# naver/multi-hmr

Hardware: NVIDIA H100
Metric: images/sec multiHMR_896_L bs=8 (higher is better)
Workload: dtype fp16 tensor-core operands, fp32 accumulate/residual

## Files before the change

### multi-hmr_b200/csrc/common.cuh

```cuda
#pragma once

#include <cuda.h>
#include <cuda_fp16.h>
#include <cuda_runtime.h>
#include <stdint.h>
#include <stdio.h>
#include <string>

#include "../../include/mhmr.h"

namespace mhmr {

__device__ __forceinline__ void griddep_launch_dependents() { asm volatile("griddepcontrol.launch_dependents;" ::: "memory"); }
__device__ __forceinline__ void griddep_wait() { asm volatile("griddepcontrol.wait;" ::: "memory"); }


void set_last_error(const std::string& msg);
const char* get_last_error();

#define MHMR_CUDA_CHECK(expr)                                                          \
  do {                                                                                 \
    cudaError_t _e = (expr);                                                           \
    if (_e != cudaSuccess) {                                                           \
      ::mhmr::set_last_error(std::string(#expr) + " failed: " + cudaGetErrorString(_e) + \
                             " at " + __FILE__ + ":" + std::to_string(__LINE__));      \
      return MHMR_ERR_CUDA;                                                    \
    }                                                                                  \
  } while (0)

#define MHMR_REQUIRE(cond, msg)                                                        \
  do {                                                                                 \
    if (!(cond)) {                                                                     \
      ::mhmr::set_last_error(std::string("requirement failed: ") + #cond + " — " + msg); \
      return MHMR_ERR_ARG;                                                     \
    }                                                                                  \
  } while (0)

#define TRY(...)                    \
  do {                              \
    int rc_ = (__VA_ARGS__);        \
    if (rc_ != MHMR_OK) return rc_; \
  } while (0)

int make_tmap_2d(CUtensorMap* out, const void* gptr, CUtensorMapDataType dtype, int elem_bytes,
                 uint64_t rows, uint64_t cols, uint64_t pitch_bytes, uint32_t box_rows,
                 uint32_t box_cols, bool swizzle128);
int make_tmap_3d(CUtensorMap* out, const void* gptr, CUtensorMapDataType dtype, int elem_bytes,
                 uint64_t depth, uint64_t rows, uint64_t cols, uint64_t depth_pitch_bytes, uint64_t pitch_bytes,
                 uint32_t box_rows, uint32_t box_cols, bool swizzle128);

int device_sm_count();
struct PerDeviceOnce {
  bool done[64] = {};
  bool first();
};
bool pdl_enabled();

#ifdef __CUDACC__
__device__ __forceinline__ uint32_t smem_u32(const void* p) {
  return static_cast<uint32_t>(__cvta_generic_to_shared(p));
}
__device__ __forceinline__ uint32_t lane_id() { return threadIdx.x & 31u; }
__device__ __forceinline__ bool elect_one_sync() {
  uint32_t pred = 0;
  asm volatile(
      "{\n\t.reg .b32 rx;\n\t.reg .pred px;\n\t"
      "elect.sync rx|px, %1;\n\t"
      "selp.u32 %0, 1, 0, px;\n\t}"
      : "=r"(pred)
      : "r"(0xffffffffu));
  return pred != 0;
}

__device__ __forceinline__ void mbar_init(uint64_t* bar, uint32_t count) {
  asm volatile("mbarrier.init.shared::cta.b64 [%0], %1;" ::"r"(smem_u32(bar)), "r"(count));
}
__device__ __forceinline__ void fence_barrier_init() {
  asm volatile("fence.mbarrier_init.release.cluster;" ::: "memory");
}
__device__ __forceinline__ void fence_proxy_async_smem() {
  asm volatile("fence.proxy.async.shared::cta;" ::: "memory");
}
__device__ __forceinline__ void mbar_arrive_expect_tx(uint64_t* bar, uint32_t bytes) {
  asm volatile("mbarrier.arrive.expect_tx.shared::cta.b64 _, [%0], %1;" ::"r"(smem_u32(bar)),
               "r"(bytes)
               : "memory");
}
__device__ __forceinline__ void mbar_arrive(uint64_t* bar) {
  asm volatile("mbarrier.arrive.shared::cta.b64 _, [%0];" ::"r"(smem_u32(bar)) : "memory");
}
__device__ __forceinline__ bool mbar_try_wait(uint64_t* bar, uint32_t parity) {
  uint32_t ok;
  asm volatile(
      "{\n\t.reg .pred p;\n\t"
      "mbarrier.try_wait.parity.shared::cta.b64 p, [%1], %2;\n\t"
      "selp.u32 %0, 1, 0, p;\n\t}"
      : "=r"(ok)
      : "r"(smem_u32(bar)), "r"(parity)
      : "memory");
  return ok != 0;
}
#ifndef MHMR_SPIN_LIMIT
#define MHMR_SPIN_LIMIT (1u << 28)
#endif
__device__ __forceinline__ void mbar_wait(uint64_t* bar, uint32_t parity) {
  uint32_t spins = 0;
  while (!mbar_try_wait(bar, parity)) {
    if (++spins > MHMR_SPIN_LIMIT) __trap();
  }
}

__device__ __forceinline__ void tma_prefetch_desc(const CUtensorMap* tmap) {
  asm volatile("prefetch.tensormap [%0];" ::"l"(reinterpret_cast<uint64_t>(tmap)) : "memory");
}
__device__ __forceinline__ void tma_load_2d(void* smem_dst, const CUtensorMap* tmap, uint64_t* bar,
                                            int32_t c_inner, int32_t c_outer) {
  asm volatile(
      "cp.async.bulk.tensor.2d.shared::cluster.global.mbarrier::complete_tx::bytes"
      " [%0], [%1, {%3, %4}], [%2];"
      :
      : "r"(smem_u32(smem_dst)), "l"(reinterpret_cast<uint64_t>(tmap)), "r"(smem_u32(bar)),
        "r"(c_inner), "r"(c_outer)
      : "memory");
}
__device__ __forceinline__ void tma_load_2d_hint(void* smem_dst, const CUtensorMap* tmap,
                                                 uint64_t* bar, int32_t c_inner, int32_t c_outer,
                                                 uint64_t cache_hint) {
  asm volatile(
      "cp.async.bulk.tensor.2d.shared::cluster.global.mbarrier::complete_tx::bytes.L2::cache_hint"
      " [%0], [%1, {%3, %4}], [%2], %5;"
      :
      : "r"(smem_u32(smem_dst)), "l"(reinterpret_cast<uint64_t>(tmap)), "r"(smem_u32(bar)),
        "r"(c_inner), "r"(c_outer), "l"(cache_hint)
      : "memory");
}
__device__ __forceinline__ void tma_load_3d_hint(void* smem_dst, const CUtensorMap* tmap, uint64_t* bar,
                                                 int32_t c_inner, int32_t c_row, int32_t c_depth,
                                                 uint64_t cache_hint) {
  asm volatile(
      "cp.async.bulk.tensor.3d.shared::cluster.global.mbarrier::complete_tx::bytes.L2::cache_hint"
      " [%0], [%1, {%3, %4, %5}], [%2], %6;"
      :
      : "r"(smem_u32(smem_dst)), "l"(reinterpret_cast<uint64_t>(tmap)), "r"(smem_u32(bar)),
        "r"(c_inner), "r"(c_row), "r"(c_depth), "l"(cache_hint)
      : "memory");
}
__device__ __forceinline__ void tma_store_2d(const CUtensorMap* tmap, const void* smem_src,
                                             int32_t c_inner, int32_t c_outer) {
  asm volatile("cp.async.bulk.tensor.2d.global.shared::cta.bulk_group [%0, {%2, %3}], [%1];"
               :
               : "l"(reinterpret_cast<uint64_t>(tmap)), "r"(smem_u32(smem_src)), "r"(c_inner),
                 "r"(c_outer)
               : "memory");
}
__device__ __forceinline__ void tma_store_commit() {
  asm volatile("cp.async.bulk.commit_group;" ::: "memory");
}
template <int N>
__device__ __forceinline__ void tma_store_wait_read() {
  asm volatile("cp.async.bulk.wait_group.read %0;" ::"n"(N) : "memory");
}
template <int N>
__device__ __forceinline__ void tma_store_wait() {
  asm volatile("cp.async.bulk.wait_group %0;" ::"n"(N) : "memory");
}
constexpr uint64_t kCacheEvictFirst = 0x12F0000000000000ull;
constexpr uint64_t kCacheEvictLast = 0x14F0000000000000ull;
constexpr uint64_t kCacheEvictNormal = 0x1000000000000000ull;

__device__ __forceinline__ uint32_t cluster_ctarank() {
  uint32_t r;
  asm volatile("mov.u32 %0, %%cluster_ctarank;" : "=r"(r));
  return r;
}
__device__ __forceinline__ void cluster_sync_all() {
  asm volatile("barrier.cluster.arrive.release.aligned;" ::: "memory");
  asm volatile("barrier.cluster.wait.acquire.aligned;" ::: "memory");
}
__device__ __forceinline__ void mbar_arrive_remote(uint64_t* bar, uint32_t cta) {
  uint32_t remote;
  asm volatile("mapa.shared::cluster.u32 %0, %1, %2;" : "=r"(remote) : "r"(smem_u32(bar)), "r"(cta));
  asm volatile("mbarrier.arrive.shared::cluster.b64 _, [%0];" ::"r"(remote) : "memory");
}
__device__ __forceinline__ void tma_load_2d_multicast(void* smem_dst, const CUtensorMap* tmap, uint64_t* bar,
                                                      int32_t c_inner, int32_t c_outer, uint16_t cta_mask) {
  asm volatile(
      "cp.async.bulk.tensor.2d.shared::cluster.global.mbarrier::complete_tx::bytes.multicast::cluster"
      " [%0], [%1, {%3, %4}], [%2], %5;"
      :
      : "r"(smem_u32(smem_dst)), "l"(reinterpret_cast<uint64_t>(tmap)), "r"(smem_u32(bar)),
        "r"(c_inner), "r"(c_outer), "h"(cta_mask)
      : "memory");
}

__device__ __forceinline__ uint64_t make_sw128_desc(uint32_t smem_addr, uint32_t lbo_bytes,
                                                    uint32_t sbo_bytes) {
  uint64_t d = 0;
  d |= static_cast<uint64_t>((smem_addr & 0x3FFFFu) >> 4);
  d |= static_cast<uint64_t>((lbo_bytes >> 4) & 0x3FFFu) << 16;
  d |= static_cast<uint64_t>((sbo_bytes >> 4) & 0x3FFFu) << 32;
  d |= 1ull << 62;
  return d;
}
__device__ __forceinline__ void wgmma_fence() { asm volatile("wgmma.fence.sync.aligned;" ::: "memory"); }
__device__ __forceinline__ void wgmma_commit() { asm volatile("wgmma.commit_group.sync.aligned;" ::: "memory"); }
template <int N>
__device__ __forceinline__ void wgmma_wait() {
  asm volatile("wgmma.wait_group.sync.aligned %0;" ::"n"(N) : "memory");
}
__device__ __forceinline__ void named_bar_sync(uint32_t id, uint32_t count) {
  asm volatile("bar.sync %0, %1;" ::"r"(id), "r"(count) : "memory");
}
__device__ __forceinline__ void named_bar_arrive(uint32_t id, uint32_t count) {
  asm volatile("bar.arrive %0, %1;" ::"r"(id), "r"(count) : "memory");
}
template <int R>
__device__ __forceinline__ void wgmma_fence_regs(float (&d)[R]) {
#pragma unroll
  for (int i = 0; i < R; ++i) asm volatile("" : "+f"(d[i])::"memory");
}

#define MHMR_WG_D8(o) "+f"(d[o + 0]), "+f"(d[o + 1]), "+f"(d[o + 2]), "+f"(d[o + 3]), \
                      "+f"(d[o + 4]), "+f"(d[o + 5]), "+f"(d[o + 6]), "+f"(d[o + 7])
__device__ __forceinline__ void wgmma_m64n64_ss(float (&d)[32], uint64_t da, uint64_t db, uint32_t acc) {
  asm volatile(
      "{\n\t.reg .pred p;\n\tsetp.ne.b32 p, %34, 0;\n\t"
      "wgmma.mma_async.sync.aligned.m64n64k16.f32.f16.f16 "
      "{%0, %1, %2, %3, %4, %5, %6, %7, %8, %9, %10, %11, %12, %13, %14, %15, "
      "%16, %17, %18, %19, %20, %21, %22, %23, %24, %25, %26, %27, %28, %29, %30, %31}, "
      "%32, %33, p, 1, 1, 0, 0;\n\t}"
      : MHMR_WG_D8(0), MHMR_WG_D8(8), MHMR_WG_D8(16), MHMR_WG_D8(24)
      : "l"(da), "l"(db), "r"(acc));
}
__device__ __forceinline__ void wgmma_m64n32_ss(float (&d)[16], uint64_t da, uint64_t db, uint32_t acc) {
  asm volatile(
      "{\n\t.reg .pred p;\n\tsetp.ne.b32 p, %18, 0;\n\t"
      "wgmma.mma_async.sync.aligned.m64n32k16.f32.f16.f16 "
      "{%0, %1, %2, %3, %4, %5, %6, %7, %8, %9, %10, %11, %12, %13, %14, %15}, "
      "%16, %17, p, 1, 1, 0, 0;\n\t}"
      : MHMR_WG_D8(0), MHMR_WG_D8(8)
      : "l"(da), "l"(db), "r"(acc));
}
__device__ __forceinline__ void wgmma_m64n128_ss(float (&d)[64], uint64_t da, uint64_t db, uint32_t acc) {
  asm volatile(
      "{\n\t.reg .pred p;\n\tsetp.ne.b32 p, %66, 0;\n\t"
      "wgmma.mma_async.sync.aligned.m64n128k16.f32.f16.f16 "
      "{%0, %1, %2, %3, %4, %5, %6, %7, %8, %9, %10, %11, %12, %13, %14, %15, "
      "%16, %17, %18, %19, %20, %21, %22, %23, %24, %25, %26, %27, %28, %29, %30, %31, "
      "%32, %33, %34, %35, %36, %37, %38, %39, %40, %41, %42, %43, %44, %45, %46, %47, "
      "%48, %49, %50, %51, %52, %53, %54, %55, %56, %57, %58, %59, %60, %61, %62, %63}, "
      "%64, %65, p, 1, 1, 0, 0;\n\t}"
      : MHMR_WG_D8(0), MHMR_WG_D8(8), MHMR_WG_D8(16), MHMR_WG_D8(24), MHMR_WG_D8(32), MHMR_WG_D8(40),
        MHMR_WG_D8(48), MHMR_WG_D8(56)
      : "l"(da), "l"(db), "r"(acc));
}
__device__ __forceinline__ void wgmma_m64n64_rs_bt(float (&d)[32], const uint32_t (&a)[4], uint64_t db) {
  asm volatile(
      "{\n\t.reg .pred p;\n\tsetp.ne.b32 p, 1, 0;\n\t"
      "wgmma.mma_async.sync.aligned.m64n64k16.f32.f16.f16 "
      "{%0, %1, %2, %3, %4, %5, %6, %7, %8, %9, %10, %11, %12, %13, %14, %15, "
      "%16, %17, %18, %19, %20, %21, %22, %23, %24, %25, %26, %27, %28, %29, %30, %31}, "
      "{%32, %33, %34, %35}, %36, p, 1, 1, 1;\n\t}"
      : MHMR_WG_D8(0), MHMR_WG_D8(8), MHMR_WG_D8(16), MHMR_WG_D8(24)
      : "r"(a[0]), "r"(a[1]), "r"(a[2]), "r"(a[3]), "l"(db));
}
#undef MHMR_WG_D8

__device__ __forceinline__ float2 fma2(float2 a, float2 b, float2 c) {
  return make_float2(fmaf(a.x, b.x, c.x), fmaf(a.y, b.y, c.y));
}
__device__ __forceinline__ float2 mul2(float2 a, float2 b) { return make_float2(__fmul_rn(a.x, b.x), __fmul_rn(a.y, b.y)); }
__device__ __forceinline__ float2 add2(float2 a, float2 b) { return make_float2(__fadd_rn(a.x, b.x), __fadd_rn(a.y, b.y)); }

__device__ __forceinline__ float gelu_erf(float x) {
  return 0.5f * x * (1.0f + erff(x * 0.70710678118654752440f));
}

__device__ __forceinline__ float gelu_erf_fast(float x) {
  const float z = fabsf(x) * 0.70710678118654752440f;
  float t;
  asm("rcp.approx.ftz.f32 %0, %1;" : "=f"(t) : "f"(fmaf(0.3275911f, z, 1.0f)));
  float e;
  asm("ex2.approx.ftz.f32 %0, %1;" : "=f"(e) : "f"(-(z * z) * 1.4426950408889634f));
  float p = fmaf(1.061405429f, t, -1.453152027f);
  p = fmaf(p, t, 1.421413741f);
  p = fmaf(p, t, -0.284496736f);
  p = fmaf(p, t, 0.254829592f);
  const float erf_abs = fmaf(-p * t, e, 1.0f);
  return 0.5f * x * (1.0f + copysignf(erf_abs, x));
}

__device__ __forceinline__ float2 gelu_erf_fast2(float2 x) {
  const float2 ax = make_float2(fabsf(x.x), fabsf(x.y));
  const float2 z = mul2(ax, make_float2(0.70710678118654752440f, 0.70710678118654752440f));
  const float2 d = fma2(z, make_float2(0.3275911f, 0.3275911f), make_float2(1.0f, 1.0f));
  float2 t, e;
  asm("rcp.approx.ftz.f32 %0, %1;" : "=f"(t.x) : "f"(d.x));
  asm("rcp.approx.ftz.f32 %0, %1;" : "=f"(t.y) : "f"(d.y));
  const float2 a = mul2(mul2(z, z), make_float2(-1.4426950408889634f, -1.4426950408889634f));
  asm("ex2.approx.ftz.f32 %0, %1;" : "=f"(e.x) : "f"(a.x));
  asm("ex2.approx.ftz.f32 %0, %1;" : "=f"(e.y) : "f"(a.y));
  float2 p = fma2(make_float2(1.061405429f, 1.061405429f), t, make_float2(-1.453152027f, -1.453152027f));
  p = fma2(p, t, make_float2(1.421413741f, 1.421413741f));
  p = fma2(p, t, make_float2(-0.284496736f, -0.284496736f));
  p = fma2(p, t, make_float2(0.254829592f, 0.254829592f));
  const float2 pte = mul2(mul2(p, t), e);
  const float2 erf_abs = fma2(pte, make_float2(-1.0f, -1.0f), make_float2(1.0f, 1.0f));
  const float2 s = make_float2(copysignf(erf_abs.x, x.x), copysignf(erf_abs.y, x.y));
  const float2 hx = mul2(x, make_float2(0.5f, 0.5f));
  return fma2(hx, s, hx);
}

__device__ __forceinline__ float warp_sum(float v) {
#pragma unroll
  for (int o = 16; o > 0; o >>= 1) v += __shfl_xor_sync(0xffffffffu, v, o);
  return v;
}
__device__ __forceinline__ float warp_max(float v) {
#pragma unroll
  for (int o = 16; o > 0; o >>= 1) v = fmaxf(v, __shfl_xor_sync(0xffffffffu, v, o));
  return v;
}
#endif

}
```

### multi-hmr_b200/csrc/gemm_epilogue.cuh

```cuda
#pragma once
#include "gemm_tc.cuh"

namespace mhmr {

constexpr int kScratchStride = 36;
constexpr int kScratchBytes = 32 * kScratchStride * 4;


struct EpiRowState {
  float sum[4], sq[4];
  float rstd;
};

template <int EPI>
constexpr bool epi_is_ln_consumer() { return EPI == EPI_LN_BIAS_F16 || EPI == EPI_LN_GELU_F16; }

struct EpiStatsPrefetch {
  float4 v[4];
};
constexpr int kMaxStatSlots = 8;

template <int EPI>
__device__ __forceinline__ void epilogue_load_row_stats(EpiStatsPrefetch& pf, const GemmEpi& ep, int M, int m_base,
                                                        int lane) {
  if constexpr (epi_is_ln_consumer<EPI>()) {
    const int m = m_base + lane;
    const float4* p = reinterpret_cast<const float4*>(ep.stats + static_cast<int64_t>(m) * ep.stat_slots);
    const int n4 = (m < M) ? (ep.stat_slots >> 1) : 0;
#pragma unroll
    for (int i = 0; i < 4; ++i) pf.v[i] = (i < n4) ? __ldcg(p + i) : make_float4(0.f, 0.f, 0.f, 0.f);
  }
}

template <int EPI>
__device__ __forceinline__ void epilogue_tile_begin(EpiRowState& st, const EpiStatsPrefetch& pf, const GemmEpi& ep,
                                                    int K) {
  if constexpr (EPI == EPI_LS_RESID_SPLIT) {
#pragma unroll
    for (int k = 0; k < 4; ++k) st.sum[k] = st.sq[k] = 0.f;
  }
  if constexpr (epi_is_ln_consumer<EPI>()) {
    const float s = (pf.v[0].x + pf.v[0].z) + (pf.v[1].x + pf.v[1].z) + (pf.v[2].x + pf.v[2].z) + (pf.v[3].x + pf.v[3].z);
    const float q = (pf.v[0].y + pf.v[0].w) + (pf.v[1].y + pf.v[1].w) + (pf.v[2].y + pf.v[2].w) + (pf.v[3].y + pf.v[3].w);
    const float inv = 1.0f / static_cast<float>(K);
    const float mean = s * inv;
    const float var = fmaxf(q * inv - mean * mean, 0.f);
    st.rstd = rsqrtf(var + ep.ln_eps);
  }
}

template <int EPI>
__device__ __forceinline__ void epilogue_tile_end(EpiRowState& st, const GemmEpi& ep, int M, int m_base, int slot,
                                                  int lane) {
  if constexpr (EPI == EPI_LS_RESID_SPLIT) {
    const int cg = lane & 3, rs = lane >> 2;
    const bool h2 = cg & 2, h1 = cg & 1;
#pragma unroll
    for (int i = 0; i < 2; ++i) {
      const float ss = h2 ? st.sum[i] : st.sum[i + 2], ks = h2 ? st.sum[i + 2] : st.sum[i];
      const float sq = h2 ? st.sq[i] : st.sq[i + 2], kq = h2 ? st.sq[i + 2] : st.sq[i];
      st.sum[i] = ks + __shfl_xor_sync(0xffffffffu, ss, 2);
      st.sq[i] = kq + __shfl_xor_sync(0xffffffffu, sq, 2);
    }
    {
      const float ss = h1 ? st.sum[0] : st.sum[1], ks = h1 ? st.sum[1] : st.sum[0];
      const float sq = h1 ? st.sq[0] : st.sq[1], kq = h1 ? st.sq[1] : st.sq[0];
      st.sum[0] = ks + __shfl_xor_sync(0xffffffffu, ss, 1);
      st.sq[0] = kq + __shfl_xor_sync(0xffffffffu, sq, 1);
    }
    const int m = m_base + cg * 8 + rs;
    if (m < M) ep.stats[static_cast<int64_t>(m) * ep.stat_slots + slot] = make_float2(st.sum[0], st.sq[0]);
  }
}

__device__ __forceinline__ void unpack_half8(const uint4& u, float (&f)[8]) {
  const __half2* h = reinterpret_cast<const __half2*>(&u);
#pragma unroll
  for (int i = 0; i < 4; ++i) {
    const float2 t = __half22float2(h[i]);
    f[2 * i] = t.x;
    f[2 * i + 1] = t.y;
  }
}

template <int EPI>
__device__ __forceinline__ void epilogue_chunk(const float* scratch, const GemmEpi& ep, int M, int N, int m_base,
                                               int n0, int lane, EpiRowState& st) {
  constexpr bool kLn = epi_is_ln_consumer<EPI>();
  constexpr bool kRowAdd16 = (EPI == EPI_ROWADD_F16);
  constexpr bool kF16 = (EPI == EPI_BIAS_F16 || EPI == EPI_BIAS_GELU_F16 || EPI == EPI_BIAS_RELU_F16 || kLn || kRowAdd16);
  constexpr bool kResid = (EPI == EPI_LS_RESID_F32);
  if constexpr (EPI == EPI_LS_RESID_SPLIT) {
    const int cg = lane & 3, rs = lane >> 2;
    const int n = n0 + cg * 8;
    float bb[8], gg[8];
    *reinterpret_cast<float4*>(bb) = __ldg(reinterpret_cast<const float4*>(ep.bias + n));
    *reinterpret_cast<float4*>(bb + 4) = __ldg(reinterpret_cast<const float4*>(ep.bias + n + 4));
    *reinterpret_cast<float4*>(gg) = __ldg(reinterpret_cast<const float4*>(ep.gamma + n));
    *reinterpret_cast<float4*>(gg + 4) = __ldg(reinterpret_cast<const float4*>(ep.gamma + n + 4));
    uint4 hi[4], lo[4];
#pragma unroll
    for (int k = 0; k < 4; ++k) {
      const int m = m_base + k * 8 + rs;
      const int64_t off = static_cast<int64_t>(m) * ep.ldx16 + n;
      hi[k] = lo[k] = make_uint4(0u, 0u, 0u, 0u);
      if (m < M) {
        hi[k] = *reinterpret_cast<const uint4*>(ep.x16 + off);
        lo[k] = *reinterpret_cast<const uint4*>(ep.xlo + off);
      }
    }
#pragma unroll
    for (int k = 0; k < 4; ++k) {
      const int rl = k * 8 + rs;
      float v[8], xh[8], xl[8], a[8];
      *reinterpret_cast<float4*>(v) = *reinterpret_cast<const float4*>(scratch + rl * kScratchStride + cg * 8);
      *reinterpret_cast<float4*>(v + 4) = *reinterpret_cast<const float4*>(scratch + rl * kScratchStride + cg * 8 + 4);
      unpack_half8(hi[k], xh);
      unpack_half8(lo[k], xl);
      float s = 0.f, q = 0.f;
      uint32_t ph[4], pl[4];
#pragma unroll
      for (int i = 0; i < 8; ++i) {
        a[i] = fmaf(gg[i], v[i] + bb[i], xh[i] + xl[i]);
        s += a[i];
        q = fmaf(a[i], a[i], q);
      }
#pragma unroll
      for (int i = 0; i < 4; ++i) {
        const __half2 h = __floats2half2_rn(a[2 * i], a[2 * i + 1]);
        const float2 hf = __half22float2(h);
        const __half2 l = __floats2half2_rn(a[2 * i] - hf.x, a[2 * i + 1] - hf.y);
        ph[i] = *reinterpret_cast<const uint32_t*>(&h);
        pl[i] = *reinterpret_cast<const uint32_t*>(&l);
      }
      st.sum[k] += s;
      st.sq[k] += q;
      if (m_base + rl < M) {
        const int64_t off = static_cast<int64_t>(m_base + rl) * ep.ldx16 + n;
        *reinterpret_cast<uint4*>(ep.x16 + off) = make_uint4(ph[0], ph[1], ph[2], ph[3]);
        *reinterpret_cast<uint4*>(ep.xlo + off) = make_uint4(pl[0], pl[1], pl[2], pl[3]);
      }
    }
  } else if constexpr (kF16) {
    const int cg = lane & 3, rs = lane >> 2;
    const int n = n0 + cg * 8;
    float4 b0 = make_float4(0.f, 0.f, 0.f, 0.f), b1 = b0;
    if constexpr (!kRowAdd16) {
      b0 = __ldg(reinterpret_cast<const float4*>(ep.bias + n));
      b1 = __ldg(reinterpret_cast<const float4*>(ep.bias + n + 4));
    }
#pragma unroll
    for (int k = 0; k < 4; ++k) {
      const int rl = k * 8 + rs;
      const int m = m_base + rl;
      if constexpr (kRowAdd16) {
        if (m < M) {
          const float* ra = ep.rowadd + static_cast<int64_t>(m % ep.rows_in) * N + n;
          b0 = __ldg(reinterpret_cast<const float4*>(ra));
          b1 = __ldg(reinterpret_cast<const float4*>(ra + 4));
        }
      }
      const float4 v0 = *reinterpret_cast<const float4*>(scratch + rl * kScratchStride + cg * 8);
      const float4 v1 = *reinterpret_cast<const float4*>(scratch + rl * kScratchStride + cg * 8 + 4);
      float2 y[4];
      if constexpr (kLn) {
        const float rstd = __shfl_sync(0xffffffffu, st.rstd, rl);
        const float2 r2 = make_float2(rstd, rstd);
        y[0] = fma2(make_float2(v0.x, v0.y), r2, make_float2(b0.x, b0.y));
        y[1] = fma2(make_float2(v0.z, v0.w), r2, make_float2(b0.z, b0.w));
        y[2] = fma2(make_float2(v1.x, v1.y), r2, make_float2(b1.x, b1.y));
        y[3] = fma2(make_float2(v1.z, v1.w), r2, make_float2(b1.z, b1.w));
      } else {
        y[0] = add2(make_float2(v0.x, v0.y), make_float2(b0.x, b0.y));
        y[1] = add2(make_float2(v0.z, v0.w), make_float2(b0.z, b0.w));
        y[2] = add2(make_float2(v1.x, v1.y), make_float2(b1.x, b1.y));
        y[3] = add2(make_float2(v1.z, v1.w), make_float2(b1.z, b1.w));
      }
#pragma unroll
      for (int i = 0; i < 4; ++i) {
        if constexpr (EPI == EPI_BIAS_GELU_F16 || EPI == EPI_LN_GELU_F16) y[i] = gelu_erf_fast2(y[i]);
        if constexpr (EPI == EPI_BIAS_RELU_F16) y[i] = make_float2(fmaxf(y[i].x, 0.0f), fmaxf(y[i].y, 0.0f));
      }
      const float x[8] = {y[0].x, y[0].y, y[1].x, y[1].y, y[2].x, y[2].y, y[3].x, y[3].y};
      const __half2 h0 = __floats2half2_rn(x[0], x[1]), h1 = __floats2half2_rn(x[2], x[3]);
      const __half2 h2 = __floats2half2_rn(x[4], x[5]), h3 = __floats2half2_rn(x[6], x[7]);
      uint4 pk;
      pk.x = *reinterpret_cast<const uint32_t*>(&h0);
      pk.y = *reinterpret_cast<const uint32_t*>(&h1);
      pk.z = *reinterpret_cast<const uint32_t*>(&h2);
      pk.w = *reinterpret_cast<const uint32_t*>(&h3);
      if (m < M)
        *reinterpret_cast<uint4*>(reinterpret_cast<__half*>(ep.out) + static_cast<int64_t>(m) * ep.ldo + n) = pk;
    }
  } else {
    const int cg = lane & 7, rs = lane >> 3;
    const int n = n0 + cg * 4;
    float4 b = make_float4(0.f, 0.f, 0.f, 0.f), g = make_float4(1.f, 1.f, 1.f, 1.f);
    if constexpr (kResid) {
      b = __ldg(reinterpret_cast<const float4*>(ep.bias + n));
      g = __ldg(reinterpret_cast<const float4*>(ep.gamma + n));
    } else if constexpr (EPI == EPI_BIAS_F32) {
      if (ep.bias != nullptr) b = __ldg(reinterpret_cast<const float4*>(ep.bias + n));
    }
    float* outp[8];
    float4 xres[8];
#pragma unroll
    for (int k = 0; k < 8; ++k) {
      const int m = m_base + k * 4 + rs;
      int64_t orow = m;
      if constexpr (EPI == EPI_ROWADD_F32) {
        const int grp = m / ep.rows_in, rin = m - grp * ep.rows_in;
        orow = static_cast<int64_t>(grp) * ep.rows_out + ep.row_off + rin;
        xres[k] = (m < M) ? __ldg(reinterpret_cast<const float4*>(ep.rowadd + static_cast<int64_t>(rin) * N + n))
                          : make_float4(0.f, 0.f, 0.f, 0.f);
      }
      outp[k] = reinterpret_cast<float*>(ep.out) + orow * ep.ldo + n;
      if constexpr (kResid)
        xres[k] = (m < M) ? *reinterpret_cast<const float4*>(outp[k]) : make_float4(0.f, 0.f, 0.f, 0.f);
    }
#pragma unroll
    for (int k = 0; k < 8; ++k) {
      const int rl = k * 4 + rs;
      const float4 v = *reinterpret_cast<const float4*>(scratch + rl * kScratchStride + cg * 4);
      float4 a;
      if constexpr (kResid) {
        a.x = xres[k].x + g.x * (v.x + b.x);
        a.y = xres[k].y + g.y * (v.y + b.y);
        a.z = xres[k].z + g.z * (v.z + b.z);
        a.w = xres[k].w + g.w * (v.w + b.w);
      } else if constexpr (EPI == EPI_ROWADD_F32) {
        a.x = v.x + xres[k].x; a.y = v.y + xres[k].y; a.z = v.z + xres[k].z; a.w = v.w + xres[k].w;
      } else {
        a.x = v.x + b.x; a.y = v.y + b.y; a.z = v.z + b.z; a.w = v.w + b.w;
      }
      if (m_base + rl < M) *reinterpret_cast<float4*>(outp[k]) = a;
    }
  }
  __syncwarp();
}

}
```

### multi-hmr_b200/csrc/gemm_tc.cu

```cuda
#include "gemm_tc.cuh"
#include "gemm_epilogue.cuh"

namespace mhmr {

namespace {

constexpr int BM = 128;
constexpr int BK = 64;
constexpr int kConsumers = 2;
constexpr int kThreads = 128 * (1 + kConsumers);
constexpr int kEpiWarps = 4 * kConsumers;
constexpr int kRegsProducer = 40, kRegsConsumer = 232;

template <int BN>
struct GemmCfg {
  static constexpr int kStages = (BN == 256) ? 3 : 5;
  static constexpr int kABytes = BM * BK * 2;
  static constexpr int kBBytes = BN * BK * 2;
  static constexpr int kStageBytes = kABytes + kBBytes;
  static constexpr int kBarBytes = 256;
  static constexpr int kSmemBytes =
      kStages * kStageBytes + kEpiWarps * kScratchBytes + kBarBytes + 1024;
  static constexpr int kAcc = BN / 4;
};

template <int NACC>
__device__ __forceinline__ void wgmma_ss(float (&d)[NACC], uint64_t da, uint64_t db, uint32_t acc) {
  if constexpr (NACC == 64) wgmma_m64n128_ss(d, da, db, acc);
  else wgmma_m64n64_ss(d, da, db, acc);
}

template <int BN, int CL, int EPI>
__global__ void __launch_bounds__(kThreads, 1)
gemm_tc_kernel(const __grid_constant__ CUtensorMap tmA, const __grid_constant__ CUtensorMap tmB,
               int M, int N, int K, GemmEpi ep) {
  using Cfg = GemmCfg<BN>;
  constexpr int kStages = Cfg::kStages;
  constexpr int kAcc = Cfg::kAcc;

  extern __shared__ uint8_t smem_raw[];
  uint8_t* smem = smem_raw + ((1024u - (smem_u32(smem_raw) & 1023u)) & 1023u);
  float* scratch_base = reinterpret_cast<float*>(smem + kStages * Cfg::kStageBytes);
  uint64_t* bars = reinterpret_cast<uint64_t*>(smem + kStages * Cfg::kStageBytes + kEpiWarps * kScratchBytes);
  uint64_t* full_bar = bars;
  uint64_t* empty_bar = bars + kStages;

  const int warp = threadIdx.x >> 5;
  const int lane = threadIdx.x & 31;
  const int wg = threadIdx.x >> 7;
  const uint32_t rank = (CL > 1) ? cluster_ctarank() : 0u;

  const int num_m = (M + BM * CL - 1) / (BM * CL);
  const int num_n = (N + BN - 1) / BN;
  const int num_tiles = num_m * num_n;
  const int num_kb = (K + BK - 1) / BK;
  const int first_tile = blockIdx.x / CL, tile_stride = gridDim.x / CL;

  griddep_launch_dependents();
  if (threadIdx.x == 0) {
    tma_prefetch_desc(&tmA);
    tma_prefetch_desc(&tmB);
    for (int s = 0; s < kStages; ++s) {
      mbar_init(&full_bar[s], 1);
      mbar_init(&empty_bar[s], kConsumers * CL);
    }
    fence_barrier_init();
  }
  if constexpr (CL > 1) cluster_sync_all();
  else __syncthreads();
  griddep_wait();

  if (wg == 0) {
    asm volatile("setmaxnreg.dec.sync.aligned.u32 %0;" ::"n"(kRegsProducer));
    if (warp == 0) {
      uint32_t stage = 0, phase = 0;
      for (int tile = first_tile; tile < num_tiles; tile += tile_stride) {
        const int m_blk = tile / num_n, n_blk = tile % num_n;
        const int row0 = m_blk * BM * CL + static_cast<int>(rank) * BM;
        for (int kb = 0; kb < num_kb; ++kb) {
          mbar_wait(&empty_bar[stage], phase ^ 1u);
          uint8_t* sa = smem + stage * Cfg::kStageBytes;
          uint8_t* sb = sa + Cfg::kABytes;
          if (elect_one_sync()) {
            mbar_arrive_expect_tx(&full_bar[stage], Cfg::kStageBytes);
            tma_load_2d(sa, &tmA, &full_bar[stage], kb * BK, row0);
            if constexpr (CL > 1) {
              constexpr int kHalf = BN / CL;
              tma_load_2d_multicast(sb + rank * (kHalf * BK * 2), &tmB, &full_bar[stage], kb * BK,
                                    n_blk * BN + static_cast<int>(rank) * kHalf, static_cast<uint16_t>((1u << CL) - 1u));
            } else {
              tma_load_2d(sb, &tmB, &full_bar[stage], kb * BK, n_blk * BN);
            }
          }
          __syncwarp();
          if (++stage == kStages) { stage = 0; phase ^= 1u; }
        }
      }
    }
  } else {
    asm volatile("setmaxnreg.inc.sync.aligned.u32 %0;" ::"n"(kRegsConsumer));
    const int cw = wg - 1;
    const int w = warp & 3;
    const bool release_lane = (threadIdx.x & 127) == 0;
    float* scratch = scratch_base + (warp - 4) * (kScratchBytes / 4);
    auto release = [&](uint32_t s) {
      if (release_lane) {
        mbar_arrive(&empty_bar[s]);
        if constexpr (CL > 1) {
#pragma unroll
          for (int c = 0; c < CL; ++c)
            if (c != static_cast<int>(rank)) mbar_arrive_remote(&empty_bar[s], static_cast<uint32_t>(c));
        }
      }
    };
    uint32_t stage = 0, phase = 0;
    EpiStatsPrefetch pf;
    auto tile_m_base = [&](int tile) { return (tile / num_n) * BM * CL + static_cast<int>(rank) * BM + 32 * w; };
    if (first_tile < num_tiles) epilogue_load_row_stats<EPI>(pf, ep, M, tile_m_base(first_tile), lane);
    for (int tile = first_tile; tile < num_tiles; tile += tile_stride) {
      const int n_blk = tile % num_n;
      const int m_base = tile_m_base(tile);
      EpiRowState rowst;
      epilogue_tile_begin<EPI>(rowst, pf, ep, K);
      if (tile + tile_stride < num_tiles)
        epilogue_load_row_stats<EPI>(pf, ep, M, tile_m_base(tile + tile_stride), lane);

      float acc[2][kAcc];
      uint32_t prev_stage = 0;
      for (int kb = 0; kb < num_kb; ++kb) {
        mbar_wait(&full_bar[stage], phase);
        const uint32_t sa = smem_u32(smem + stage * Cfg::kStageBytes);
        const uint32_t sb = sa + Cfg::kABytes + cw * (BN / 2) * (BK * 2);
        const uint64_t a_desc0 = make_sw128_desc(sa, 16, 2048);
        const uint64_t a_desc1 = make_sw128_desc(sa + 1024, 16, 2048);
        const uint64_t b_desc = make_sw128_desc(sb, 16, 1024);
        wgmma_fence();
#pragma unroll
        for (int k = 0; k < BK / 16; ++k) {
          const uint32_t accumulate = (kb > 0 || k > 0) ? 1u : 0u;
          wgmma_ss<kAcc>(acc[0], a_desc0 + 2u * k, b_desc + 2u * k, accumulate);
          wgmma_ss<kAcc>(acc[1], a_desc1 + 2u * k, b_desc + 2u * k, accumulate);
        }
        wgmma_commit();
        wgmma_wait<1>();
        if (kb > 0) release(prev_stage);
        prev_stage = stage;
        if (++stage == kStages) { stage = 0; phase ^= 1u; }
      }
      wgmma_wait<0>();
      wgmma_fence_regs(acc[0]);
      wgmma_fence_regs(acc[1]);
      release(prev_stage);

#pragma unroll
      for (int c = 0; c < BN / 64; ++c) {
#pragma unroll
        for (int h = 0; h < 2; ++h)
#pragma unroll
          for (int g = 0; g < 4; ++g)
#pragma unroll
            for (int rr = 0; rr < 2; ++rr) {
              const int i = 4 * (4 * c + g) + 2 * rr;
              const int r = (lane >> 2) + 8 * h + 16 * rr;
              *reinterpret_cast<float2*>(scratch + r * kScratchStride + g * 8 + 2 * (lane & 3)) =
                  make_float2(acc[h][i], acc[h][i + 1]);
            }
        __syncwarp();
        const int n0 = n_blk * BN + cw * (BN / 2) + c * 32;
        if (n0 < N) epilogue_chunk<EPI>(scratch, ep, M, N, m_base, n0, lane, rowst);
        __syncwarp();
      }
      epilogue_tile_end<EPI>(rowst, ep, M, m_base, n_blk * kConsumers + cw, lane);
    }
  }
  if constexpr (CL > 1) cluster_sync_all();
}

template <int BN, int CL, int EPI>
int launch_one(const GemmPlan* p, cudaStream_t stream) {
  using Cfg = GemmCfg<BN>;
  auto kern = gemm_tc_kernel<BN, CL, EPI>;
  static PerDeviceOnce once;
  if (once.first()) {
    MHMR_CUDA_CHECK(cudaFuncSetAttribute(kern, cudaFuncAttributeMaxDynamicSharedMemorySize,
                                         Cfg::kSmemBytes));
  }
  cudaLaunchConfig_t cfg{};
  cfg.gridDim = dim3(p->grid);
  cfg.blockDim = dim3(kThreads);
  cfg.dynamicSmemBytes = Cfg::kSmemBytes;
  cfg.stream = stream;
  cudaLaunchAttribute attr[2];
  int n = 0;
  if (CL > 1) {
    attr[n].id = cudaLaunchAttributeClusterDimension;
    attr[n].val.clusterDim.x = CL;
    attr[n].val.clusterDim.y = 1;
    attr[n].val.clusterDim.z = 1;
    ++n;
  }
  if (pdl_enabled()) {
    attr[n].id = cudaLaunchAttributeProgrammaticStreamSerialization;
    attr[n].val.programmaticStreamSerializationAllowed = 1;
    ++n;
  }
  cfg.attrs = attr;
  cfg.numAttrs = n;
  MHMR_CUDA_CHECK(cudaLaunchKernelEx(&cfg, kern, p->tmA, p->tmB, p->M, p->N, p->K, p->ep));
  return MHMR_OK;
}

template <int BN, int CL>
int launch_bn(const GemmPlan* p, cudaStream_t stream) {
  switch (p->epi) {
    case EPI_BIAS_F16: return launch_one<BN, CL, EPI_BIAS_F16>(p, stream);
    case EPI_BIAS_GELU_F16: return launch_one<BN, CL, EPI_BIAS_GELU_F16>(p, stream);
    case EPI_BIAS_RELU_F16: return launch_one<BN, CL, EPI_BIAS_RELU_F16>(p, stream);
    case EPI_LS_RESID_F32: return launch_one<BN, CL, EPI_LS_RESID_F32>(p, stream);
    case EPI_ROWADD_F32: return launch_one<BN, CL, EPI_ROWADD_F32>(p, stream);
    case EPI_BIAS_F32: return launch_one<BN, CL, EPI_BIAS_F32>(p, stream);
    case EPI_LS_RESID_SPLIT: return launch_one<BN, CL, EPI_LS_RESID_SPLIT>(p, stream);
    case EPI_LN_BIAS_F16: return launch_one<BN, CL, EPI_LN_BIAS_F16>(p, stream);
    case EPI_LN_GELU_F16: return launch_one<BN, CL, EPI_LN_GELU_F16>(p, stream);
    case EPI_ROWADD_F16: return launch_one<BN, CL, EPI_ROWADD_F16>(p, stream);
    default: break;
  }
  set_last_error("gemm: unknown epilogue kind");
  return MHMR_ERR_ARG;
}

}

int gemm_plan_init(GemmPlan* plan, const __half* A, int64_t lda, const __half* W, int64_t ldw, int M,
                   int N, int K, int epi_kind, const GemmEpi& ep, int bn) {
  MHMR_REQUIRE(M > 0 && N > 0 && K > 0, "gemm: empty problem");
  MHMR_REQUIRE(N % 32 == 0, "gemm: N must be a multiple of 32");
  MHMR_REQUIRE(lda % 8 == 0 && ldw % 8 == 0, "gemm: row pitches must be multiples of 8 fp16 (16 B, TMA)");
  MHMR_REQUIRE((reinterpret_cast<uintptr_t>(A) & 15) == 0 && (reinterpret_cast<uintptr_t>(W) & 15) == 0,
               "gemm: operands must be 16-byte aligned");
  MHMR_REQUIRE(bn == 128 || bn == 256 || bn == 512, "gemm: block_n must be 128, 256 or 512 (CTA pair)");
  MHMR_REQUIRE(epi_kind >= 0 && epi_kind < EPI_NUM_KINDS, "gemm: bad epilogue kind");
  if (epi_kind != EPI_LS_RESID_SPLIT)
    MHMR_REQUIRE(ep.out != nullptr && ep.ldo % 8 == 0, "gemm: output missing or pitch not multiple of 8");
  if (epi_kind != EPI_BIAS_F32 && epi_kind != EPI_ROWADD_F32 && epi_kind != EPI_ROWADD_F16)
    MHMR_REQUIRE(ep.bias != nullptr, "gemm: bias required for this epilogue");
  if (epi_kind == EPI_LS_RESID_F32 || epi_kind == EPI_LS_RESID_SPLIT)
    MHMR_REQUIRE(ep.gamma != nullptr, "gemm: gamma required");
  if (epi_kind == EPI_LS_RESID_SPLIT)
    MHMR_REQUIRE(ep.x16 != nullptr && ep.xlo != nullptr && ep.ldx16 % 8 == 0 && ep.stats != nullptr &&
                     ep.stat_slots == gemm_stat_slots(N, bn) && N % (bn == 128 ? 128 : 256) == 0,
                 "gemm: split-stream epilogue needs both planes, stats, whole column tiles and matching slot count");
  if (epi_kind == EPI_LN_BIAS_F16 || epi_kind == EPI_LN_GELU_F16)
    MHMR_REQUIRE(ep.stats != nullptr && ep.stat_slots > 0 && ep.stat_slots % 2 == 0 && ep.stat_slots <= 8,
                 "gemm: folded-LN consumer needs row statistics (even slot count, at most 8)");
  if (epi_kind == EPI_ROWADD_F32 || epi_kind == EPI_ROWADD_F16)
    MHMR_REQUIRE(ep.rowadd != nullptr && ep.rows_in > 0, "gemm: rowadd/rows_in required");
  plan->M = M; plan->N = N; plan->K = K; plan->bn = bn; plan->epi = epi_kind; plan->ep = ep;
  int rc = make_tmap_2d(&plan->tmA, A, CU_TENSOR_MAP_DATA_TYPE_FLOAT16, 2, M, K, lda * 2, BM, BK, true);
  if (rc != MHMR_OK) return rc;
  rc = make_tmap_2d(&plan->tmB, W, CU_TENSOR_MAP_DATA_TYPE_FLOAT16, 2, N, K, ldw * 2, bn == 512 ? 128 : bn, BK,
                    true);
  if (rc != MHMR_OK) return rc;
  plan->grid = gemm_plan_grid(plan, M);
  return MHMR_OK;
}

int gemm_plan_grid(const GemmPlan* plan, int M) {
  const int sms = device_sm_count();
  if (plan->bn == 512) {
    const int tiles = ((M + 255) / 256) * ((plan->N + 255) / 256);
    const int pairs = sms / 2;
    return 2 * (tiles < pairs ? tiles : pairs);
  }
  const int tiles = ((M + BM - 1) / BM) * ((plan->N + plan->bn - 1) / plan->bn);
  return tiles < sms ? tiles : sms;
}

int gemm_stat_slots(int N, int bn) {
  const int tile_n = (bn == 128) ? 128 : 256;
  return ((N + tile_n - 1) / tile_n) * kConsumers;
}

int gemm_plan_run(const GemmPlan* plan, cudaStream_t stream) {
  if (plan->bn == 512) return launch_bn<256, 2>(plan, stream);
  return plan->bn == 256 ? launch_bn<256, 1>(plan, stream) : launch_bn<128, 1>(plan, stream);
}

int gemm_plan_run_rows(const GemmPlan* plan, int M, cudaStream_t stream) {
  MHMR_REQUIRE(M > 0 && M <= plan->M, "gemm: a plan runs at most the rows it was built for");
  GemmPlan p = *plan;
  p.M = M;
  p.grid = gemm_plan_grid(&p, M);
  return gemm_plan_run(&p, stream);
}

}
```

Baseline: 80.19.

## Split GEMM tile across consumers by rows with one wide wgmma per consumer

Each consumer warpgroup now owns 64 rows across the full BN width and issues a single m64nBNk16 wgmma per k-step, instead of splitting columns and issuing two m64n(BN/2) wgmmas over 128 rows. The epilogue is reworked for 16-row warp slices, and the per-row LayerNorm statistic slots are remapped to two per tile. The intent is fewer, wider wgmma instructions that reuse the A fragment better and lower issue overhead. In exchange the B tile is read by both consumers, and the epilogue and stats bookkeeping change, which risks register pressure and correctness in the split-stat path.

After: 81.11, median of 6. +1.1%, better.

```diff
diff --git a/multi-hmr_b200/csrc/common.cuh b/multi-hmr_b200/csrc/common.cuh
--- a/multi-hmr_b200/csrc/common.cuh
+++ b/multi-hmr_b200/csrc/common.cuh
@@ -252,6 +252,24 @@
       "%64, %65, p, 1, 1, 0, 0;\n\t}"
       : MHMR_WG_D8(0), MHMR_WG_D8(8), MHMR_WG_D8(16), MHMR_WG_D8(24), MHMR_WG_D8(32), MHMR_WG_D8(40),
         MHMR_WG_D8(48), MHMR_WG_D8(56)
+      : "l"(da), "l"(db), "r"(acc));
+}
+__device__ __forceinline__ void wgmma_m64n256_ss(float (&d)[128], uint64_t da, uint64_t db, uint32_t acc) {
+  asm volatile(
+      "{\n\t.reg .pred p;\n\tsetp.ne.b32 p, %130, 0;\n\t"
+      "wgmma.mma_async.sync.aligned.m64n256k16.f32.f16.f16 "
+      "{%0, %1, %2, %3, %4, %5, %6, %7, %8, %9, %10, %11, %12, %13, %14, %15, "
+      "%16, %17, %18, %19, %20, %21, %22, %23, %24, %25, %26, %27, %28, %29, %30, %31, "
+      "%32, %33, %34, %35, %36, %37, %38, %39, %40, %41, %42, %43, %44, %45, %46, %47, "
+      "%48, %49, %50, %51, %52, %53, %54, %55, %56, %57, %58, %59, %60, %61, %62, %63, "
+      "%64, %65, %66, %67, %68, %69, %70, %71, %72, %73, %74, %75, %76, %77, %78, %79, "
+      "%80, %81, %82, %83, %84, %85, %86, %87, %88, %89, %90, %91, %92, %93, %94, %95, "
+      "%96, %97, %98, %99, %100, %101, %102, %103, %104, %105, %106, %107, %108, %109, %110, %111, "
+      "%112, %113, %114, %115, %116, %117, %118, %119, %120, %121, %122, %123, %124, %125, %126, %127}, "
+      "%128, %129, p, 1, 1, 0, 0;\n\t}"
+      : MHMR_WG_D8(0), MHMR_WG_D8(8), MHMR_WG_D8(16), MHMR_WG_D8(24), MHMR_WG_D8(32), MHMR_WG_D8(40),
+        MHMR_WG_D8(48), MHMR_WG_D8(56), MHMR_WG_D8(64), MHMR_WG_D8(72), MHMR_WG_D8(80), MHMR_WG_D8(88),
+        MHMR_WG_D8(96), MHMR_WG_D8(104), MHMR_WG_D8(112), MHMR_WG_D8(120)
       : "l"(da), "l"(db), "r"(acc));
 }
 __device__ __forceinline__ void wgmma_m64n64_rs_bt(float (&d)[32], const uint32_t (&a)[4], uint64_t db) {
diff --git a/multi-hmr_b200/csrc/gemm_epilogue.cuh b/multi-hmr_b200/csrc/gemm_epilogue.cuh
--- a/multi-hmr_b200/csrc/gemm_epilogue.cuh
+++ b/multi-hmr_b200/csrc/gemm_epilogue.cuh
@@ -3,8 +3,9 @@
 
 namespace mhmr {
 
+constexpr int kEpiRows = 16;
 constexpr int kScratchStride = 36;
-constexpr int kScratchBytes = 32 * kScratchStride * 4;
+constexpr int kScratchBytes = kEpiRows * kScratchStride * 4;
 
 
 struct EpiRowState {
@@ -24,7 +25,7 @@
 __device__ __forceinline__ void epilogue_load_row_stats(EpiStatsPrefetch& pf, const GemmEpi& ep, int M, int m_base,
                                                         int lane) {
   if constexpr (epi_is_ln_consumer<EPI>()) {
-    const int m = m_base + lane;
+    const int m = m_base + (lane & (kEpiRows - 1));
     const float4* p = reinterpret_cast<const float4*>(ep.stats + static_cast<int64_t>(m) * ep.stat_slots);
     const int n4 = (m < M) ? (ep.stat_slots >> 1) : 0;
 #pragma unroll
@@ -50,7 +51,7 @@
 }
 
 template <int EPI>
-__device__ __forceinline__ void epilogue_tile_end(EpiRowState& st, const GemmEpi& ep, int M, int m_base, int slot,
+__device__ __forceinline__ void epilogue_tile_end(EpiRowState& st, const GemmEpi& ep, int M, int m_base, int slot0,
                                                   int lane) {
   if constexpr (EPI == EPI_LS_RESID_SPLIT) {
     const int cg = lane & 3, rs = lane >> 2;
@@ -68,8 +69,8 @@
       st.sum[0] = ks + __shfl_xor_sync(0xffffffffu, ss, 1);
       st.sq[0] = kq + __shfl_xor_sync(0xffffffffu, sq, 1);
     }
-    const int m = m_base + cg * 8 + rs;
-    if (m < M) ep.stats[static_cast<int64_t>(m) * ep.stat_slots + slot] = make_float2(st.sum[0], st.sq[0]);
+    const int m = m_base + (cg & 1) * 8 + rs;
+    if (m < M) ep.stats[static_cast<int64_t>(m) * ep.stat_slots + slot0 + (cg >> 1)] = make_float2(st.sum[0], st.sq[0]);
   }
 }
 
@@ -85,7 +86,7 @@
 
 template <int EPI>
 __device__ __forceinline__ void epilogue_chunk(const float* scratch, const GemmEpi& ep, int M, int N, int m_base,
-                                               int n0, int lane, EpiRowState& st) {
+                                               int n0, int half, int lane, EpiRowState& st) {
   constexpr bool kLn = epi_is_ln_consumer<EPI>();
   constexpr bool kRowAdd16 = (EPI == EPI_ROWADD_F16);
   constexpr bool kF16 = (EPI == EPI_BIAS_F16 || EPI == EPI_BIAS_GELU_F16 || EPI == EPI_BIAS_RELU_F16 || kLn || kRowAdd16);
@@ -98,9 +99,9 @@
     *reinterpret_cast<float4*>(bb + 4) = __ldg(reinterpret_cast<const float4*>(ep.bias + n + 4));
     *reinterpret_cast<float4*>(gg) = __ldg(reinterpret_cast<const float4*>(ep.gamma + n));
     *reinterpret_cast<float4*>(gg + 4) = __ldg(reinterpret_cast<const float4*>(ep.gamma + n + 4));
-    uint4 hi[4], lo[4];
-#pragma unroll
-    for (int k = 0; k < 4; ++k) {
+    uint4 hi[2], lo[2];
+#pragma unroll
+    for (int k = 0; k < 2; ++k) {
       const int m = m_base + k * 8 + rs;
       const int64_t off = static_cast<int64_t>(m) * ep.ldx16 + n;
       hi[k] = lo[k] = make_uint4(0u, 0u, 0u, 0u);
@@ -110,7 +111,7 @@
       }
     }
 #pragma unroll
-    for (int k = 0; k < 4; ++k) {
+    for (int k = 0; k < 2; ++k) {
       const int rl = k * 8 + rs;
       float v[8], xh[8], xl[8], a[8];
       *reinterpret_cast<float4*>(v) = *reinterpret_cast<const float4*>(scratch + rl * kScratchStride + cg * 8);
@@ -133,8 +134,8 @@
         ph[i] = *reinterpret_cast<const uint32_t*>(&h);
         pl[i] = *reinterpret_cast<const uint32_t*>(&l);
       }
-      st.sum[k] += s;
-      st.sq[k] += q;
+      st.sum[2 * half + k] += s;
+      st.sq[2 * half + k] += q;
       if (m_base + rl < M) {
         const int64_t off = static_cast<int64_t>(m_base + rl) * ep.ldx16 + n;
         *reinterpret_cast<uint4*>(ep.x16 + off) = make_uint4(ph[0], ph[1], ph[2], ph[3]);
@@ -150,7 +151,7 @@
       b1 = __ldg(reinterpret_cast<const float4*>(ep.bias + n + 4));
     }
 #pragma unroll
-    for (int k = 0; k < 4; ++k) {
+    for (int k = 0; k < 2; ++k) {
       const int rl = k * 8 + rs;
       const int m = m_base + rl;
       if constexpr (kRowAdd16) {
@@ -202,10 +203,10 @@
     } else if constexpr (EPI == EPI_BIAS_F32) {
       if (ep.bias != nullptr) b = __ldg(reinterpret_cast<const float4*>(ep.bias + n));
     }
-    float* outp[8];
-    float4 xres[8];
-#pragma unroll
-    for (int k = 0; k < 8; ++k) {
+    float* outp[4];
+    float4 xres[4];
+#pragma unroll
+    for (int k = 0; k < 4; ++k) {
       const int m = m_base + k * 4 + rs;
       int64_t orow = m;
       if constexpr (EPI == EPI_ROWADD_F32) {
@@ -219,7 +220,7 @@
         xres[k] = (m < M) ? *reinterpret_cast<const float4*>(outp[k]) : make_float4(0.f, 0.f, 0.f, 0.f);
     }
 #pragma unroll
-    for (int k = 0; k < 8; ++k) {
+    for (int k = 0; k < 4; ++k) {
       const int rl = k * 4 + rs;
       const float4 v = *reinterpret_cast<const float4*>(scratch + rl * kScratchStride + cg * 4);
       float4 a;
diff --git a/multi-hmr_b200/csrc/gemm_tc.cu b/multi-hmr_b200/csrc/gemm_tc.cu
--- a/multi-hmr_b200/csrc/gemm_tc.cu
+++ b/multi-hmr_b200/csrc/gemm_tc.cu
@@ -11,6 +11,7 @@
 constexpr int kThreads = 128 * (1 + kConsumers);
 constexpr int kEpiWarps = 4 * kConsumers;
 constexpr int kRegsProducer = 40, kRegsConsumer = 232;
+constexpr int kSlotsPerTile = 2;
 
 template <int BN>
 struct GemmCfg {
@@ -21,13 +22,14 @@
   static constexpr int kBarBytes = 256;
   static constexpr int kSmemBytes =
       kStages * kStageBytes + kEpiWarps * kScratchBytes + kBarBytes + 1024;
-  static constexpr int kAcc = BN / 4;
+  static constexpr int kAcc = BN / 2;
+  static_assert(kSmemBytes <= 227 * 1024, "operand ring + epilogue scratch exceed the shared memory of an SM");
 };
 
 template <int NACC>
 __device__ __forceinline__ void wgmma_ss(float (&d)[NACC], uint64_t da, uint64_t db, uint32_t acc) {
-  if constexpr (NACC == 64) wgmma_m64n128_ss(d, da, db, acc);
-  else wgmma_m64n64_ss(d, da, db, acc);
+  if constexpr (NACC == 128) wgmma_m64n256_ss(d, da, db, acc);
+  else wgmma_m64n128_ss(d, da, db, acc);
 }
 
 template <int BN, int CL, int EPI>
@@ -115,7 +117,9 @@
     };
     uint32_t stage = 0, phase = 0;
     EpiStatsPrefetch pf;
-    auto tile_m_base = [&](int tile) { return (tile / num_n) * BM * CL + static_cast<int>(rank) * BM + 32 * w; };
+    auto tile_m_base = [&](int tile) {
+      return (tile / num_n) * BM * CL + static_cast<int>(rank) * BM + 64 * cw + kEpiRows * w;
+    };
     if (first_tile < num_tiles) epilogue_load_row_stats<EPI>(pf, ep, M, tile_m_base(first_tile), lane);
     for (int tile = first_tile; tile < num_tiles; tile += tile_stride) {
       const int n_blk = tile % num_n;
@@ -125,21 +129,18 @@
       if (tile + tile_stride < num_tiles)
         epilogue_load_row_stats<EPI>(pf, ep, M, tile_m_base(tile + tile_stride), lane);
 
-      float acc[2][kAcc];
+      float acc[kAcc];
       uint32_t prev_stage = 0;
       for (int kb = 0; kb < num_kb; ++kb) {
         mbar_wait(&full_bar[stage], phase);
         const uint32_t sa = smem_u32(smem + stage * Cfg::kStageBytes);
-        const uint32_t sb = sa + Cfg::kABytes + cw * (BN / 2) * (BK * 2);
-        const uint64_t a_desc0 = make_sw128_desc(sa, 16, 2048);
-        const uint64_t a_desc1 = make_sw128_desc(sa + 1024, 16, 2048);
-        const uint64_t b_desc = make_sw128_desc(sb, 16, 1024);
+        const uint64_t a_desc = make_sw128_desc(sa + cw * 64 * (BK * 2), 16, 1024);
+        const uint64_t b_desc = make_sw128_desc(sa + Cfg::kABytes, 16, 1024);
         wgmma_fence();
 #pragma unroll
         for (int k = 0; k < BK / 16; ++k) {
           const uint32_t accumulate = (kb > 0 || k > 0) ? 1u : 0u;
-          wgmma_ss<kAcc>(acc[0], a_desc0 + 2u * k, b_desc + 2u * k, accumulate);
-          wgmma_ss<kAcc>(acc[1], a_desc1 + 2u * k, b_desc + 2u * k, accumulate);
+          wgmma_ss<kAcc>(acc, a_desc + 2u * k, b_desc + 2u * k, accumulate);
         }
         wgmma_commit();
         wgmma_wait<1>();
@@ -148,29 +149,26 @@
         if (++stage == kStages) { stage = 0; phase ^= 1u; }
       }
       wgmma_wait<0>();
-      wgmma_fence_regs(acc[0]);
-      wgmma_fence_regs(acc[1]);
+      wgmma_fence_regs(acc);
       release(prev_stage);
 
 #pragma unroll
-      for (int c = 0; c < BN / 64; ++c) {
-#pragma unroll
-        for (int h = 0; h < 2; ++h)
-#pragma unroll
-          for (int g = 0; g < 4; ++g)
-#pragma unroll
-            for (int rr = 0; rr < 2; ++rr) {
-              const int i = 4 * (4 * c + g) + 2 * rr;
-              const int r = (lane >> 2) + 8 * h + 16 * rr;
-              *reinterpret_cast<float2*>(scratch + r * kScratchStride + g * 8 + 2 * (lane & 3)) =
-                  make_float2(acc[h][i], acc[h][i + 1]);
-            }
+      for (int c = 0; c < BN / 32; ++c) {
+#pragma unroll
+        for (int g = 0; g < 4; ++g)
+#pragma unroll
+          for (int rr = 0; rr < 2; ++rr) {
+            const int i = 4 * (4 * c + g) + 2 * rr;
+            const int r = (lane >> 2) + 8 * rr;
+            *reinterpret_cast<float2*>(scratch + r * kScratchStride + g * 8 + 2 * (lane & 3)) =
+                make_float2(acc[i], acc[i + 1]);
+          }
         __syncwarp();
-        const int n0 = n_blk * BN + cw * (BN / 2) + c * 32;
-        if (n0 < N) epilogue_chunk<EPI>(scratch, ep, M, N, m_base, n0, lane, rowst);
+        const int n0 = n_blk * BN + c * 32;
+        if (n0 < N) epilogue_chunk<EPI>(scratch, ep, M, N, m_base, n0, c / (BN / 64), lane, rowst);
         __syncwarp();
       }
-      epilogue_tile_end<EPI>(rowst, ep, M, m_base, n_blk * kConsumers + cw, lane);
+      epilogue_tile_end<EPI>(rowst, ep, M, m_base, n_blk * kSlotsPerTile, lane);
     }
   }
   if constexpr (CL > 1) cluster_sync_all();
@@ -278,7 +276,7 @@
 
 int gemm_stat_slots(int N, int bn) {
   const int tile_n = (bn == 128) ? 128 : 256;
-  return ((N + tile_n - 1) / tile_n) * kConsumers;
+  return ((N + tile_n - 1) / tile_n) * kSlotsPerTile;
 }
 
 int gemm_plan_run(const GemmPlan* plan, cudaStream_t stream) {
```
